# intel/hexl

Measured on NVIDIA H100. Metric: ntt_per_sec_fwd_inv_N65536_q55_batch8192, higher is better.
Workload: dtype u64

## Files before the change

### hexl_b200/csrc/ntt.cu

```cuda
#include "ntt_kernels.cuh"

namespace hexl_b200 {
namespace {

template <int MODE, int LOGC>
cudaError_t launch_row(bool fwd, const NttDeviceTables& t, u64* result, const u64* operand,
                       u64 batch, int out_mf, int fold, cudaStream_t stream) {
  using Cfg = RowCfg<LOGC, MODE>;
  const unsigned rows_per_poly = (unsigned)(t.n >> LOGC);
  const u64 total_rows = batch * rows_per_poly;
  const unsigned grid = (unsigned)((total_rows + Cfg::ROWS - 1) / Cfg::ROWS);
  const Mod m = make_mod(t);
  if (fwd) {
    if (cudaError_t e = ensure_dynamic_smem<ntt_row_fwd<MODE, LOGC>>(Cfg::SMEM)) return e;
    ntt_row_fwd<MODE, LOGC><<<grid, Cfg::THREADS, Cfg::SMEM, stream>>>(result, operand, Tab<MODE>::fwd(t), m,
                                                                       total_rows, rows_per_poly, out_mf);
  } else {
    if (cudaError_t e = ensure_dynamic_smem<ntt_row_inv<MODE, LOGC>>(Cfg::SMEM)) return e;
    ntt_row_inv<MODE, LOGC><<<grid, Cfg::THREADS, Cfg::SMEM, stream>>>(
        result, operand, Tab<MODE>::inv(t), m, total_rows, rows_per_poly, out_mf, fold, Tab<MODE>::inv_n(t),
        Tab<MODE>::inv_n_w(t));
  }
  count_launch();
  return cudaGetLastError();
}

template <int MODE>
cudaError_t launch_row_dyn(int log_c, bool fwd, const NttDeviceTables& t, u64* result,
                           const u64* operand, u64 batch, int out_mf, int fold,
                           cudaStream_t stream) {
  switch (log_c) {
#define ROW_CASE(L) \
  case L: return launch_row<MODE, L>(fwd, t, result, operand, batch, out_mf, fold, stream);
    ROW_CASE(4) ROW_CASE(5) ROW_CASE(6) ROW_CASE(7) ROW_CASE(8) ROW_CASE(9) ROW_CASE(10)
    ROW_CASE(11) ROW_CASE(12) ROW_CASE(13)
#undef ROW_CASE
  }
  return cudaErrorInvalidValue;
}

template <int MODE, int LOGR>
cudaError_t launch_col(bool fwd, const NttDeviceTables& t, u64* result, const u64* operand,
                       u64 batch, int log_s, int out_mf, int fold, cudaStream_t stream) {
  const u64 total_cols = (batch << t.log_n) >> LOGR;
  const u64 cols_per_block = 1ull << (log_s - LOGR);
  const unsigned threads = (unsigned)(cols_per_block < 256 ? cols_per_block : 256);
  const unsigned grid = (unsigned)((total_cols + threads - 1) / threads);
  const Mod m = make_mod(t);
  if (fwd)
    ntt_col<MODE, LOGR, true><<<grid, threads, 0, stream>>>(result, operand, Tab<MODE>::fwd(t), m, t.log_n, log_s,
                                                            total_cols, out_mf, fold, Tab<MODE>::inv_n(t),
                                                            Tab<MODE>::inv_n_w(t));
  else
    ntt_col<MODE, LOGR, false><<<grid, threads, 0, stream>>>(result, operand, Tab<MODE>::inv(t), m, t.log_n, log_s,
                                                             total_cols, out_mf, fold, Tab<MODE>::inv_n(t),
                                                             Tab<MODE>::inv_n_w(t));
  count_launch();
  return cudaGetLastError();
}

template <int MODE>
cudaError_t launch_col_dyn(int log_r, bool fwd, const NttDeviceTables& t, u64* result,
                           const u64* operand, u64 batch, int log_s, int out_mf, int fold,
                           cudaStream_t stream) {
  switch (log_r) {
    case 3: return launch_col<MODE, 3>(fwd, t, result, operand, batch, log_s, out_mf, fold, stream);
    case 4: return launch_col<MODE, 4>(fwd, t, result, operand, batch, log_s, out_mf, fold, stream);
  }
  if constexpr (MODE != kSmall)
    if (log_r == 5) return launch_col<MODE, 5>(fwd, t, result, operand, batch, log_s, out_mf, fold, stream);
  return cudaErrorInvalidValue;
}

cudaError_t simple_transform(bool fwd, const NttDeviceTables& t, u64* result, const u64* operand,
                             int out_mf, u64 batch, cudaStream_t stream) {
  const u64 total = batch << (t.log_n - 1);
  const unsigned threads = 128, grid = (unsigned)((total + threads - 1) / threads);
  const u64* src = operand;
  const Mod m = make_mod(t);
  for (int k = 0; k < t.log_n; ++k) {
    const int s = fwd ? k : t.log_n - 1 - k;
    const int last = k == t.log_n - 1;
    if (fwd)
      ntt_stage_simple<true><<<grid, threads, 0, stream>>>(result, src, t.fwd, m, t.log_n, s, total,
                                                           out_mf, last, t.inv_n, t.inv_n_w);
    else
      ntt_stage_simple<false><<<grid, threads, 0, stream>>>(result, src, t.inv, m, t.log_n, s, total,
                                                            out_mf, last, t.inv_n, t.inv_n_w);
    count_launch();
    src = result;
  }
  return cudaGetLastError();
}

template <int MODE, int LOGR>
cudaError_t launch_fused(bool fwd, const NttDeviceTables& t, u64* result, const u64* operand, u64 batch,
                         int out_mf, cudaStream_t stream) {
  using Cfg = FusedCfg<LOGR>;
  const Mod m = make_mod(t);
  cudaLaunchConfig_t cfg = {};
  cfg.gridDim = dim3((unsigned)(batch * Cfg::K));
  cfg.blockDim = dim3(Cfg::THREADS);
  cfg.dynamicSmemBytes = Cfg::SMEM;
  cfg.stream = stream;
  cudaLaunchAttribute attr;
  attr.id = cudaLaunchAttributeClusterDimension;
  attr.val.clusterDim.x = Cfg::K;
  attr.val.clusterDim.y = 1;
  attr.val.clusterDim.z = 1;
  cfg.attrs = &attr;
  cfg.numAttrs = 1;
  cudaError_t e;
  if (fwd)
    e = cudaLaunchKernelEx(&cfg, ntt_fused_fwd<MODE, LOGR>, result, operand, Tab<MODE>::fwd(t), m, out_mf);
  else
    e = cudaLaunchKernelEx(&cfg, ntt_fused_inv<MODE, LOGR>, result, operand, Tab<MODE>::inv(t), m, out_mf,
                           Tab<MODE>::inv_n(t), Tab<MODE>::inv_n_w(t));
  count_launch();
  return e != cudaSuccess ? e : cudaGetLastError();
}

template <int MODE, int LOGR>
cudaError_t launch_pipe(const NttDeviceTables& t, u64* result, const u64* operand, u64 batch, int out_mf,
                        cudaStream_t stream) {
  return launch_pipelined<ntt_pipe_fwd<MODE, LOGR>, PipeCfg<LOGR>>(batch, stream, result, operand, Tab<MODE>::fwd(t),
                                                                  make_mod(t), out_mf);
}

template <int MODE, int LOGR>
cudaError_t launch_dsmem(bool fwd, const NttDeviceTables& t, u64* result, const u64* operand, u64 batch, int out_mf,
                         cudaStream_t stream) {
  using Cfg = DsmemCfg<LOGR, MODE>;
  const Mod m = make_mod(t);
  cudaLaunchConfig_t cfg = {};
  cfg.gridDim = dim3((unsigned)(batch * Cfg::K));
  cfg.blockDim = dim3(Cfg::THREADS);
  cfg.dynamicSmemBytes = Cfg::SMEM;
  cfg.stream = stream;
  cudaLaunchAttribute attr;
  attr.id = cudaLaunchAttributeClusterDimension;
  attr.val.clusterDim.x = Cfg::K;
  attr.val.clusterDim.y = 1;
  attr.val.clusterDim.z = 1;
  cfg.attrs = &attr;
  cfg.numAttrs = 1;
  cudaError_t e;
  if (fwd) {
    if ((e = ensure_dynamic_smem<ntt_dsmem_fwd<MODE, LOGR>>(Cfg::SMEM)) != cudaSuccess) return e;
    e = cudaLaunchKernelEx(&cfg, ntt_dsmem_fwd<MODE, LOGR>, result, operand, Tab<MODE>::fwd(t), m, out_mf);
  } else {
    if ((e = ensure_dynamic_smem<ntt_dsmem_inv<MODE, LOGR>>(Cfg::SMEM)) != cudaSuccess) return e;
    e = cudaLaunchKernelEx(&cfg, ntt_dsmem_inv<MODE, LOGR>, result, operand, Tab<MODE>::inv(t), m, out_mf,
                           Tab<MODE>::inv_n(t), Tab<MODE>::inv_n_w(t));
  }
  count_launch();
  return e != cudaSuccess ? e : cudaGetLastError();
}

enum : int { kSplit, kPipe, kFused, kDsmem };
struct SinglePass {
  int kernel, log_r;
};
template <int MODE>
SinglePass plan_single_pass(int log_n, u64 batch, bool forward) {
  const int lr = log_n - 12;
  if (lr < 2 || lr > 5) return {kSplit, 0};
  if (MODE == kSmall) return {kDsmem, lr};
  if (forward && lr >= 3 && batch >= 64 && batch < (1ull << 31)) return {kPipe, lr};
  if (lr <= 3) return {kDsmem, lr};
  if (lr == 4) return {kFused, lr};
  return {kSplit, 0};
}

template <int MODE>
cudaError_t launch_single_pass(SinglePass p, bool fwd, const NttDeviceTables& t, u64* result, const u64* operand,
                               u64 batch, int out_mf, cudaStream_t stream) {
  if constexpr (MODE == kSmall) {
    switch (p.log_r) {
      case 2: return launch_dsmem<MODE, 2>(fwd, t, result, operand, batch, out_mf, stream);
      case 3: return launch_dsmem<MODE, 3>(fwd, t, result, operand, batch, out_mf, stream);
      case 4: return launch_dsmem<MODE, 4>(fwd, t, result, operand, batch, out_mf, stream);
      case 5: return launch_dsmem<MODE, 5>(fwd, t, result, operand, batch, out_mf, stream);
    }
  } else if (p.kernel == kPipe && fwd) {
    switch (p.log_r) {
      case 3: return launch_pipe<MODE, 3>(t, result, operand, batch, out_mf, stream);
      case 4: return launch_pipe<MODE, 4>(t, result, operand, batch, out_mf, stream);
      case 5: return launch_pipe<MODE, 5>(t, result, operand, batch, out_mf, stream);
    }
  } else if (p.kernel == kFused && p.log_r == 4) {
    return launch_fused<MODE, 4>(fwd, t, result, operand, batch, out_mf, stream);
  } else if (p.kernel == kDsmem) {
    switch (p.log_r) {
      case 2: return launch_dsmem<MODE, 2>(fwd, t, result, operand, batch, out_mf, stream);
      case 3: return launch_dsmem<MODE, 3>(fwd, t, result, operand, batch, out_mf, stream);
    }
  }
  return cudaErrorInvalidValue;
}

template <int MODE>
cudaError_t forward_impl(const NttDeviceTables& t, u64* result, const u64* operand, int out_mf,
                         u64 batch, cudaStream_t stream) {
  const SinglePass sp = plan_single_pass<MODE>(t.log_n, batch, true);
  if (sp.kernel != kSplit) return launch_single_pass<MODE>(sp, true, t, result, operand, batch, out_mf, stream);
  const int log_c = pick_row_log(t.log_n);
  int radices[8];
  const int ncol = plan_col_passes(t.log_n - log_c, radices);
  const u64* src = operand;
  int log_s = t.log_n;
  for (int p = 0; p < ncol; ++p) {
    cudaError_t e = launch_col_dyn<MODE>(radices[p], true, t, result, src, batch, log_s, out_mf, 0, stream);
    if (e != cudaSuccess) return e;
    log_s -= radices[p];
    src = result;
  }
  return launch_row_dyn<MODE>(log_c, true, t, result, src, batch, out_mf, 0, stream);
}

template <int MODE>
cudaError_t inverse_impl(const NttDeviceTables& t, u64* result, const u64* operand, int out_mf,
                         u64 batch, cudaStream_t stream) {
  const SinglePass sp = plan_single_pass<MODE>(t.log_n, batch, false);
  if (sp.kernel != kSplit) return launch_single_pass<MODE>(sp, false, t, result, operand, batch, out_mf, stream);
  const int log_c = pick_row_log(t.log_n);
  int radices[8];
  const int ncol = plan_col_passes(t.log_n - log_c, radices);
  cudaError_t e = launch_row_dyn<MODE>(log_c, false, t, result, operand, batch, out_mf, ncol == 0, stream);
  if (e != cudaSuccess) return e;
  int log_s = log_c;
  for (int p = ncol - 1; p >= 0; --p) {
    log_s += radices[p];
    e = launch_col_dyn<MODE>(radices[p], false, t, result, result, batch, log_s, out_mf, p == 0, stream);
    if (e != cudaSuccess) return e;
  }
  return cudaSuccess;
}

}

cudaError_t launch_ntt_forward(const NttDeviceTables& t, u64* result, const u64* operand,
                               int , int out_mf, u64 batch, cudaStream_t stream) {
  if (batch == 0) return cudaSuccess;
  if (t.log_n < 4) return simple_transform(true, t, result, operand, out_mf, batch, stream);
  switch (pick_mode(t.q)) {
    case kFast: return forward_impl<kFast>(t, result, operand, out_mf, batch, stream);
    case kSmall: return forward_impl<kSmall>(t, result, operand, out_mf, batch, stream);
    case kWide: return forward_impl<kWide>(t, result, operand, out_mf, batch, stream);
  }
  return forward_impl<kGeneric>(t, result, operand, out_mf, batch, stream);
}

cudaError_t launch_ntt_inverse(const NttDeviceTables& t, u64* result, const u64* operand,
                               int , int out_mf, u64 batch, cudaStream_t stream) {
  if (batch == 0) return cudaSuccess;
  if (t.log_n < 4) return simple_transform(false, t, result, operand, out_mf, batch, stream);
  switch (pick_mode(t.q)) {
    case kFast: return inverse_impl<kFast>(t, result, operand, out_mf, batch, stream);
    case kSmall: return inverse_impl<kSmall>(t, result, operand, out_mf, batch, stream);
    case kWide: return inverse_impl<kWide>(t, result, operand, out_mf, batch, stream);
  }
  return inverse_impl<kGeneric>(t, result, operand, out_mf, batch, stream);
}

}
```

### hexl_b200/csrc/ntt_kernels.cuh

```cuda
#pragma once
#include <algorithm>
#include <atomic>
#include <cstdio>
#include <cstdlib>

#include "internal.h"

namespace hexl_b200 {
namespace {

template <int I>
struct Idx {
  __host__ __device__ constexpr operator int() const { return I; }
};
template <int BEGIN, int END, typename F>
__device__ __forceinline__ void static_for(F&& f) {
  if constexpr (BEGIN < END) {
    f(Idx<BEGIN>{});
    static_for<BEGIN + 1, END>(f);
  }
}

enum : int { kGeneric = 0, kFast = 1, kSmall = 2, kWide = 3 };

// ... 453 lines not shown
template <int POLICY>
__device__ __forceinline__ void st_coef(u64* p, u64 v) {
  if (POLICY == kViaL2)
    __stcg(p, v);
  else
    __stcs(p, v);
}

template <int POLICY, typename E>
__device__ __forceinline__ E ld_row(const void* base, unsigned u0, unsigned off) {
  const unsigned idx = u0 + off;
  if constexpr (POLICY == kSmemRow)
    return static_cast<const E*>(base)[idx];
  else if constexpr (POLICY == kSmemRowPad)
    return static_cast<const E*>(base)[idx + (idx >> 4)];
  else
    return (E)ld_coef<POLICY>(static_cast<const u64*>(base) + u0 + off);
}
template <int POLICY, typename E>
__device__ __forceinline__ void st_row(void* base, unsigned u0, unsigned off, E v) {
  const unsigned idx = u0 + off;
  if constexpr (POLICY == kSmemRow)
    static_cast<E*>(base)[idx] = v;
  else if constexpr (POLICY == kSmemRowPad)
    static_cast<E*>(base)[idx + (idx >> 4)] = v;
  else
    st_coef<POLICY>(static_cast<u64*>(base) + u0 + off, v);
}

struct MirrorList {
  u64* const* p;
  unsigned count;
  u64 off;
};

template <int MODE, int LOGC, int LD, int ST>
__device__ __forceinline__ void row_fwd_body(void* out, const void* in, typename Ar<MODE>::E* srow, unsigned u,
                                             u64 base, const typename Ar<MODE>::Tw* __restrict__ tw, const Mod& m,
                                             int out_mf, bool active, typename Ar<MODE>::Tw* cta_stab = nullptr,
                                             bool reduce_in = false) {
  using E = typename Ar<MODE>::E;
  using Tw = typename Ar<MODE>::Tw;
  E v[16];
  constexpr int LB0 = LOGC - 4;
  Tw* stab = cta_stab ? cta_stab : reinterpret_cast<Tw*>(srow + row_elems<E>(LOGC));
  const unsigned u_in = reg_index<LB0>(u, 0);
  static_for<0, 16>([&](auto I) { constexpr int e = I; v[e] = ld_row<LD, E>(in, u_in, e << LB0); });
  if constexpr (LD < kSmemRow && sizeof(E) == 8) {
    if (reduce_in) {
      static_for<0, 16>([&](auto I) { constexpr int e = I; v[e] = reduce_any(v[e], m); });
    }
  }
  if constexpr (RowCfg<LOGC>::TW_TABLES) {
    if (cta_stab)
      load_row_twiddles<LOGC>(stab, threadIdx.x, blockDim.x, base, tw);
    else
      load_row_twiddles<LOGC>(stab, u, (1u << LOGC) / 16, base, tw);
    __syncthreads();
  }
  reg_stages<MODE, LOGC, LB0, LOGC - 1, LB0, true>(v, u, base, tw, stab, m, false, Tw{}, Tw{});
  fwd_passes<MODE, LOGC, 1>(v, srow, u, base, tw, stab, m);
  static_for<0, 16>([&](auto I) { constexpr int e = I; v[e] = fwd_out<MODE>(v[e], m, out_mf); });
  constexpr int LB_OUT = LB0 < 4 ? LB0 : 4;
  if constexpr (LOGC > 4) smem_exchange<0, LB_OUT>(v, srow, u);
  if (active) {
    const unsigned u_out = reg_index<LB_OUT>(u, 0);
    static_for<0, 16>([&](auto I) { constexpr int e = I; st_row<ST, E>(out, u_out, e << LB_OUT, v[e]); });
  }
}

template <int MODE, int LOGC, int LD, int ST>
__device__ __forceinline__ void row_inv_body(void* out, const void* in, typename Ar<MODE>::E* srow, unsigned u,
                                             u64 base, const typename Ar<MODE>::Tw* __restrict__ tw, const Mod& m,
                                             int out_mf, bool fold, typename Ar<MODE>::Tw inv_n,
                                             typename Ar<MODE>::Tw inv_n_w, bool active,
                                             typename Ar<MODE>::Tw* cta_stab = nullptr, const MirrorList* mir = nullptr,
                                             const ProdIn* prod = nullptr) {
  using Cfg = RowCfg<LOGC>;
  using E = typename Ar<MODE>::E;
  using Tw = typename Ar<MODE>::Tw;
  E v[16];
  constexpr int LB0 = LOGC - 4;
  constexpr int LB_IN = LB0 < 4 ? LB0 : 4;
  Tw* stab = cta_stab ? cta_stab : reinterpret_cast<Tw*>(srow + row_elems<E>(LOGC));
  const unsigned u_in = reg_index<LB_IN>(u, 0);
  static_for<0, 16>([&](auto I) { constexpr int e = I; v[e] = ld_row<LD, E>(in, u_in, e << LB_IN); });
  if constexpr (LD < kSmemRow && sizeof(E) == 8) {
    if (prod) {
      static_for<0, 16>([&](auto I) {
        constexpr int e = I;
        v[e] = prod_lazy<MODE>(v[e], ld_coef<LD>(prod->b + reg_index<LB_IN>(u, e)), m, prod->mu, prod->shift);
      });
    }
  }
  if constexpr (Cfg::TW_TABLES) {
    if (cta_stab)
      load_row_twiddles<LOGC>(stab, threadIdx.x, blockDim.x, base, tw);
    else
      load_row_twiddles<LOGC>(stab, u, (1u << LOGC) / 16, base, tw);
    __syncthreads();
  }
  if constexpr (LOGC > 4) smem_exchange<LB_IN, 0>(v, srow, u);
  inv_passes<MODE, LOGC, Cfg::PASSES - 1>(v, srow, u, base, tw, stab, m, fold, inv_n, inv_n_w);
  if (active) {
    static_for<0, 16>([&](auto I) {
      constexpr int e = I;
      st_row<ST, E>(out, reg_index<LB0>(u, 0), e << LB0, fold ? inv_out<MODE>(v[e], m, out_mf) : v[e]);
    });
    if (mir && fold) {
      for (unsigned p = 0; p < mir->count; ++p) {
        static_for<0, 16>([&](auto I) {
          constexpr int e = I;
          mir->p[p][mir->off + reg_index<LB0>(u, e)] = (u64)inv_out<MODE>(v[e], m, out_mf);
        });
      }
    }
  }
}

template <int MODE, int LOGC>
__global__ void __launch_bounds__(RowCfg<LOGC, MODE>::THREADS, RowCfg<LOGC, MODE>::MIN_BLOCKS)
    ntt_row_fwd(u64* result, const u64* operand, const typename Ar<MODE>::Tw* __restrict__ tw, const Mod m,
                u64 total_rows, unsigned rows_per_poly, int out_mf) {
  using Cfg = RowCfg<LOGC, MODE>;
  extern __shared__ __align__(16) unsigned char smem[];
  const unsigned row_local = threadIdx.x / Cfg::T, u = threadIdx.x % Cfg::T;
  u64 row = (u64)blockIdx.x * Cfg::ROWS + row_local;
  const bool active = row < total_rows;
  if (!active) row = total_rows - 1;
  const u64 base = (u64)rows_per_poly + (row % rows_per_poly);
  typename Cfg::Tw* cta_stab = nullptr;
  if (MODE == kSmall && Cfg::ROWS > 1 && Cfg::TW_TABLES && rows_per_poly == 1)
    cta_stab = reinterpret_cast<typename Cfg::Tw*>(smem + (size_t)row_elems<typename Cfg::E>(LOGC) * sizeof(typename Cfg::E));
  row_fwd_body<MODE, LOGC, kStream, kStream>(
      result + row * Cfg::C, operand + row * Cfg::C,
      reinterpret_cast<typename Cfg::E*>(smem + (size_t)row_local * Cfg::ROW_BYTES), u, base, tw, m, out_mf, active,
      cta_stab);
}

template <int MODE, int LOGC>
__global__ void __launch_bounds__(RowCfg<LOGC, MODE>::THREADS, RowCfg<LOGC, MODE>::MIN_BLOCKS)
    ntt_row_inv(u64* result, const u64* operand, const typename Ar<MODE>::Tw* __restrict__ tw, const Mod m,
                u64 total_rows, unsigned rows_per_poly, int out_mf, int fold, typename Ar<MODE>::Tw inv_n,
                typename Ar<MODE>::Tw inv_n_w) {
  using Cfg = RowCfg<LOGC, MODE>;
  extern __shared__ __align__(16) unsigned char smem[];
  const unsigned row_local = threadIdx.x / Cfg::T, u = threadIdx.x % Cfg::T;
  u64 row = (u64)blockIdx.x * Cfg::ROWS + row_local;
  const bool active = row < total_rows;
  if (!active) row = total_rows - 1;
  const u64 base = (u64)rows_per_poly + (row % rows_per_poly);
  typename Cfg::Tw* cta_stab = nullptr;
  if (MODE == kSmall && Cfg::ROWS > 1 && Cfg::TW_TABLES && rows_per_poly == 1)
    cta_stab = reinterpret_cast<typename Cfg::Tw*>(smem + (size_t)row_elems<typename Cfg::E>(LOGC) * sizeof(typename Cfg::E));
  row_inv_body<MODE, LOGC, kStream, kStream>(
      result + row * Cfg::C, operand + row * Cfg::C,
      reinterpret_cast<typename Cfg::E*>(smem + (size_t)row_local * Cfg::ROW_BYTES), u, base, tw, m, out_mf,
      fold != 0, inv_n, inv_n_w, active, cta_stab);
}

template <int MODE, int LOGR, bool FWD>
__device__ __forceinline__ void col_stages(typename Ar<MODE>::E (&v)[1 << LOGR], const typename Ar<MODE>::Tw* stw,
                                           const Mod& m, bool root_fold, typename Ar<MODE>::Tw inv_n,
                                           typename Ar<MODE>::Tw inv_n_w) {
  using E = typename Ar<MODE>::E;
  using Tw = typename Ar<MODE>::Tw;
  constexpr int R = 1 << LOGR;
  static_for<0, LOGR>([&](auto STEP) {
    constexpr int step = STEP;
    constexpr int s = FWD ? step : LOGR - 1 - step;
    constexpr int eb = LOGR - 1 - s;
    const E cq = stage_cq<MODE>(step, m);
    auto groups = [&] {
      static_for<0, (1 << s)>([&](auto GI) {
        constexpr int gi = GI;
        const Tw w = stw[(1 << s) + gi];
        static_for<0, (1 << eb)>([&](auto L) {
          constexpr int e = (gi << (eb + 1)) | L;
          if constexpr (FWD)
            fwd_bfly<MODE>(v[e], v[e | (1 << eb)], w, m);
          else
            inv_bfly<MODE>(v[e], v[e | (1 << eb)], w, m, cq);
        });
      });
    };
    if constexpr (!FWD && s == 0) {
      if (root_fold) {
        static_for<0, (1 << eb)>([&](auto L) {
          constexpr int l = L;
          inv_bfly_last<MODE>(v[l], v[l | (1 << eb)], inv_n, inv_n_w, m, cq);
        });
      } else {
        groups();
      }
    } else {
      groups();
    }
  });
  if constexpr (!FWD && MODE == kFast) {
    if (!root_fold) inv_pass_fixup<LOGR, R>(v, m);
  }
}

template <int MODE, int LOGR, bool FWD, int LD, int ST>
__device__ __forceinline__ void col_body(u64* result, const u64* operand, u64 off, int log_stride,
                                         const typename Ar<MODE>::Tw* stw, const Mod& m, int out_mf, bool root_fold,
                                         typename Ar<MODE>::Tw inv_n, typename Ar<MODE>::Tw inv_n_w,
                                         const MirrorList* mir = nullptr, bool reduce_in = false) {
  using E = typename Ar<MODE>::E;
  constexpr int R = 1 << LOGR;
  E v[R];
  static_for<0, R>([&](auto I) {
    constexpr int e = I;
    v[e] = (E)ld_coef<LD>(operand + off + ((u64)e << log_stride));
  });
  if constexpr (FWD && sizeof(E) == 8) {
    if (reduce_in) {
      static_for<0, R>([&](auto I) { constexpr int e = I; v[e] = reduce_any(v[e], m); });
    }
  }
  col_stages<MODE, LOGR, FWD>(v, stw, m, root_fold, inv_n, inv_n_w);
  const bool final_out = !FWD && root_fold;
  static_for<0, R>([&](auto I) {
    constexpr int e = I;
    st_coef<ST>(result + off + ((u64)e << log_stride), final_out ? inv_out<MODE>(v[e], m, out_mf) : v[e]);
  });
  if (mir && final_out) {
    for (unsigned p = 0; p < mir->count; ++p) {
      static_for<0, R>([&](auto I) {
        constexpr int e = I;
        mir->p[p][mir->off + off + ((u64)e << log_stride)] = (u64)inv_out<MODE>(v[e], m, out_mf);
      });
    }
  }
}

template <int MODE, int LOGR, bool FWD>
__global__ void __launch_bounds__(256)
    ntt_col(u64* result, const u64* operand, const typename Ar<MODE>::Tw* __restrict__ tw, const Mod m, int log_n,
            int log_s, u64 total_cols, int out_mf, int fold, typename Ar<MODE>::Tw inv_n,
            typename Ar<MODE>::Tw inv_n_w) {
  constexpr int R = 1 << LOGR;
  __shared__ typename Ar<MODE>::Tw stw[R];
  const int log_cols = log_s - LOGR;
  const u64 g0 = (u64)blockIdx.x * blockDim.x;
  const u64 blk = g0 >> log_cols;
  const u64 blocks_per_poly = 1ull << (log_n - log_s);
  const u64 base = blocks_per_poly + (blk & (blocks_per_poly - 1));
  for (int l = threadIdx.x; l < R; l += blockDim.x) {
    if (l == 0) continue;
    const int s = 31 - __clz(l);
    stw[l] = ld_tw(tw + (base << s) + (l - (1 << s)));
  }
  __syncthreads();
  const u64 g = g0 + threadIdx.x;
  if (g >= total_cols) return;
  const u64 c = g & ((1ull << log_cols) - 1);
  col_body<MODE, LOGR, FWD, kStream, kStream>(result, operand, (blk << log_s) + c, log_cols, stw, m, out_mf,
                                              !FWD && fold && log_s == log_n, inv_n, inv_n_w);
}

__device__ __forceinline__ void cluster_barrier() {
  asm volatile("barrier.cluster.arrive.release.aligned;\n\tbarrier.cluster.wait.acquire.aligned;" ::: "memory");
}

template <int LOGR>
struct FusedCfg {
  static constexpr int LOGC = 12, C = 1 << LOGC, R = 1 << LOGR;
  static constexpr int K = R < 8 ? R : 8;
  static constexpr int THREADS = 256;
  static constexpr int MIN_BLOCKS = LOGR <= 4 ? kRowMinBlocks : 2;
  static constexpr size_t SMEM = RowCfg<LOGC>::ROW_BYTES;
};

template <int MODE, int LOGR>
__global__ void __launch_bounds__(FusedCfg<LOGR>::THREADS, FusedCfg<LOGR>::MIN_BLOCKS)
    ntt_fused_fwd(u64* result, const u64* operand, const typename Ar<MODE>::Tw* __restrict__ tw, const Mod m,
                  int out_mf) {
  using Cfg = FusedCfg<LOGR>;
  using E = typename Ar<MODE>::E;
  using Tw = typename Ar<MODE>::Tw;
  extern __shared__ __align__(16) unsigned char smem_raw[];
  E* smem = reinterpret_cast<E*>(smem_raw);
  __shared__ Tw stw[Cfg::R];
  const unsigned rank = blockIdx.x % Cfg::K;
  const u64 poly_off = (u64)(blockIdx.x / Cfg::K) << (Cfg::LOGC + LOGR);
  for (int l = threadIdx.x; l < Cfg::R; l += Cfg::THREADS)
    if (l) stw[l] = ld_tw(tw + l);
  __syncthreads();
  constexpr int COLS = Cfg::C / Cfg::K;
#pragma unroll 1
  for (int c = threadIdx.x; c < COLS; c += Cfg::THREADS)
    col_body<MODE, LOGR, true, kStream, kViaL2>(result, operand, poly_off + rank * COLS + c, Cfg::LOGC, stw, m,
                                                out_mf, false, Tw{}, Tw{});
  cluster_barrier();
#pragma unroll 1
  for (unsigned r = rank; r < Cfg::R; r += Cfg::K) {
    u64* row = result + poly_off + (u64)r * Cfg::C;
    row_fwd_body<MODE, Cfg::LOGC, kViaL2, kStream>(row, row, smem, threadIdx.x, (u64)Cfg::R + r, tw, m, out_mf, true);
    if (r + Cfg::K < Cfg::R) __syncthreads();
  }
}

template <int MODE, int LOGR>
__global__ void __launch_bounds__(FusedCfg<LOGR>::THREADS, FusedCfg<LOGR>::MIN_BLOCKS)
    ntt_fused_inv(u64* result, const u64* operand, const typename Ar<MODE>::Tw* __restrict__ tw, const Mod m,
                  int out_mf, typename Ar<MODE>::Tw inv_n, typename Ar<MODE>::Tw inv_n_w) {
  using Cfg = FusedCfg<LOGR>;
  using E = typename Ar<MODE>::E;
  using Tw = typename Ar<MODE>::Tw;
  extern __shared__ __align__(16) unsigned char smem_raw[];
  E* smem = reinterpret_cast<E*>(smem_raw);
  __shared__ Tw stw[Cfg::R];
  const unsigned rank = blockIdx.x % Cfg::K;
  const u64 poly_off = (u64)(blockIdx.x / Cfg::K) << (Cfg::LOGC + LOGR);
  for (int l = threadIdx.x; l < Cfg::R; l += Cfg::THREADS)
    if (l) stw[l] = ld_tw(tw + l);
#pragma unroll 1
  for (unsigned r = rank; r < Cfg::R; r += Cfg::K) {
    const u64 off = poly_off + (u64)r * Cfg::C;
    row_inv_body<MODE, Cfg::LOGC, kStream, kViaL2>(result + off, operand + off, smem, threadIdx.x, (u64)Cfg::R + r,
                                                   tw, m, out_mf, false, inv_n, inv_n_w, true);
    __syncthreads();
  }
  cluster_barrier();
  constexpr int COLS = Cfg::C / Cfg::K;
#pragma unroll 1
  for (int c = threadIdx.x; c < COLS; c += Cfg::THREADS)
    col_body<MODE, LOGR, false, kViaL2, kStream>(result, result, poly_off + rank * COLS + c, Cfg::LOGC, stw, m,
                                                 out_mf, true, inv_n, inv_n_w);
}

__device__ __forceinline__ unsigned ld_acquire_gpu(const unsigned* p) {
  unsigned v;
  asm volatile("ld.acquire.gpu.global.u32 %0, [%1];" : "=r"(v) : "l"(p) : "memory");
  return v;
}
__device__ __forceinline__ void red_release_gpu(unsigned* p, unsigned v) {
  asm volatile("red.release.gpu.global.add.u32 [%0], %1;" ::"l"(p), "r"(v) : "memory");
}

template <int LOGR>
struct PipeCfg {
  static constexpr int LOGC = 12, C = 1 << LOGC, R = 1 << LOGR;
  static constexpr int THREADS = 256;
  static constexpr int CT = C / THREADS;
  static constexpr int SLOTS = CT + R;
  static constexpr int MIN_BLOCKS = FusedCfg<LOGR>::MIN_BLOCKS;
  static constexpr size_t SMEM = RowCfg<LOGC>::ROW_BYTES;
};

template <int MODE, int LOGR>
__global__ void __launch_bounds__(PipeCfg<LOGR>::THREADS, PipeCfg<LOGR>::MIN_BLOCKS)
    ntt_pipe_fwd(u64* result, const u64* operand, const typename Ar<MODE>::Tw* __restrict__ tw, const Mod m,
                 int out_mf, unsigned batch, unsigned lookahead, unsigned* counter, unsigned* done) {
  using Cfg = PipeCfg<LOGR>;
  using E = typename Ar<MODE>::E;
  using Tw = typename Ar<MODE>::Tw;
  extern __shared__ __align__(16) unsigned char smem_raw[];
  E* smem = reinterpret_cast<E*>(smem_raw);
  __shared__ Tw stw[Cfg::R];
  __shared__ unsigned s_item;
  for (int l = threadIdx.x; l < Cfg::R; l += Cfg::THREADS)
    if (l) stw[l] = ld_tw(tw + l);
  const unsigned total = (batch + lookahead) * Cfg::SLOTS;
  while (true) {
    __syncthreads();
    if (threadIdx.x == 0) s_item = atomicAdd(counter, 1u);
    __syncthreads();
    const unsigned item = s_item;
    if (item >= total) break;
    const unsigned blk = item / Cfg::SLOTS, j = item % Cfg::SLOTS;
    if (j < (unsigned)Cfg::CT) {
      if (blk >= batch) continue;
      const u64 poly_off = (u64)blk << (Cfg::LOGC + LOGR);
      col_body<MODE, LOGR, true, kStream, kViaL2>(result, operand, poly_off + j * Cfg::THREADS + threadIdx.x, Cfg::LOGC,
                                                  stw, m, out_mf, false, Tw{}, Tw{});
      __syncthreads();
      if (threadIdx.x == 0) red_release_gpu(done + blk, 1u);
    } else {
      if (blk < lookahead) continue;
      const unsigned p = blk - lookahead, r = j - Cfg::CT;
      if (threadIdx.x == 0)
        while (ld_acquire_gpu(done + p) < (unsigned)Cfg::CT) __nanosleep(100);
      __syncthreads();
      u64* row = result + ((u64)p << (Cfg::LOGC + LOGR)) + (u64)r * Cfg::C;
      row_fwd_body<MODE, Cfg::LOGC, kViaL2, kStream>(row, row, smem, threadIdx.x, (u64)Cfg::R + r, tw, m, out_mf, true);
    }
  }
}

__device__ __forceinline__ unsigned dsmem_address(const void* local_smem, unsigned cta_rank) {
  const unsigned a = (unsigned)__cvta_generic_to_shared(local_smem);
  unsigned r;
  asm("mapa.shared::cluster.u32 %0, %1, %2;" : "=r"(r) : "r"(a), "r"(cta_rank));
  return r;
}
__device__ __forceinline__ void dsmem_store(unsigned addr, unsigned v) {
  asm volatile("st.shared::cluster.u32 [%0], %1;" ::"r"(addr), "r"(v) : "memory");
}
__device__ __forceinline__ void dsmem_store(unsigned addr, u64 v) {
  asm volatile("st.shared::cluster.u64 [%0], %1;" ::"r"(addr), "l"(v) : "memory");
}
template <typename E>
__device__ __forceinline__ E dsmem_load(unsigned addr) {
  E v;
  if constexpr (sizeof(E) == 8)
    asm volatile("ld.shared::cluster.u64 %0, [%1];" : "=l"(v) : "r"(addr) : "memory");
  else
    asm volatile("ld.shared::cluster.u32 %0, [%1];" : "=r"(v) : "r"(addr) : "memory");
  return v;
}

template <int LOGR, int MODE = kSmall>
struct DsmemCfg {
  using E = typename Ar<MODE>::E;
  using Tw = typename Ar<MODE>::Tw;
  static constexpr int LOGC = 12, C = 1 << LOGC, R = 1 << LOGR;
  static constexpr int K = R < 8 ? R : 8;
  static constexpr int RPC = R / K;
  static constexpr int THREADS = 256;
  static constexpr int COLS = C / K;
  static constexpr bool PAD = sizeof(E) == 8;
  static constexpr int ROW_POLICY = PAD ? kSmemRowPad : kSmemRow;
  static constexpr unsigned ROW = row_elems<E>(LOGC);
  static constexpr size_t SMEM = (size_t)(RPC + (PAD ? 0 : 1)) * ROW * sizeof(E) + kRowTwEntries * sizeof(Tw);
  static constexpr int MIN_BLOCKS = PAD ? kRowMinBlocks : (SMEM <= 56 * 1024 ? 4 : (SMEM <= 75 * 1024 ? 3 : 2));
  static __device__ __forceinline__ unsigned slot(unsigned j) { return PAD ? j + (j >> 4) : j; }
};

template <int MODE, int LOGR>
__global__ void __launch_bounds__(DsmemCfg<LOGR, MODE>::THREADS, DsmemCfg<LOGR, MODE>::MIN_BLOCKS)
    ntt_dsmem_fwd(u64* result, const u64* operand, const typename Ar<MODE>::Tw* __restrict__ tw, const Mod m,
                  int out_mf) {
  using Cfg = DsmemCfg<LOGR, MODE>;
  using E = typename Ar<MODE>::E;
  using Tw = typename Ar<MODE>::Tw;
  extern __shared__ __align__(16) unsigned char smem_raw[];
  E* rows = reinterpret_cast<E*>(smem_raw);
  E* xbuf = rows + Cfg::RPC * Cfg::ROW;
  Tw* const ctab = Cfg::PAD ? reinterpret_cast<Tw*>(xbuf) : nullptr;
  __shared__ Tw stw[Cfg::R];
  const unsigned rank = blockIdx.x % Cfg::K;
  const u64 poly_off = (u64)(blockIdx.x / Cfg::K) << (Cfg::LOGC + LOGR);
  asm volatile("barrier.cluster.arrive.relaxed.aligned;" ::: "memory");
  for (int l = threadIdx.x; l < Cfg::R; l += Cfg::THREADS)
    if (l) stw[l] = ld_tw(tw + l);
  __syncthreads();
  asm volatile("barrier.cluster.wait.aligned;" ::: "memory");
  unsigned owner_base[Cfg::K];
  static_for<0, Cfg::K>([&](auto I) { constexpr int o = I; owner_base[o] = dsmem_address(rows, o); });
#pragma unroll 1
  for (int c = threadIdx.x; c < Cfg::COLS; c += Cfg::THREADS) {
    const unsigned col = rank * Cfg::COLS + c;
    E v[Cfg::R];
    static_for<0, Cfg::R>([&](auto I) {
      constexpr int e = I;
      v[e] = (E)ld_coef<kStream>(operand + poly_off + ((u64)e << Cfg::LOGC) + col);
    });
    col_stages<MODE, LOGR, true>(v, stw, m, false, Tw{}, Tw{});
    static_for<0, Cfg::R>([&](auto I) {
      constexpr int e = I;
      dsmem_store(owner_base[e % Cfg::K] + ((e / Cfg::K) * Cfg::ROW + Cfg::slot(col)) * (unsigned)sizeof(E), v[e]);
    });
  }
  cluster_barrier();
#pragma unroll 1
  for (int lr = 0; lr < Cfg::RPC; ++lr) {
    const unsigned r = rank + lr * Cfg::K;
    E* row = rows + lr * Cfg::ROW;
    row_fwd_body<MODE, Cfg::LOGC, Cfg::ROW_POLICY, kStream>(result + poly_off + (u64)r * Cfg::C, row,
                                                            Cfg::PAD ? row : xbuf, threadIdx.x, (u64)Cfg::R + r, tw, m,
                                                            out_mf, true, ctab);
    if (lr + 1 < Cfg::RPC) __syncthreads();
  }
}

template <int MODE, int LOGR>
__global__ void __launch_bounds__(DsmemCfg<LOGR, MODE>::THREADS, DsmemCfg<LOGR, MODE>::MIN_BLOCKS)
    ntt_dsmem_inv(u64* result, const u64* operand, const typename Ar<MODE>::Tw* __restrict__ tw, const Mod m,
                  int out_mf, typename Ar<MODE>::Tw inv_n, typename Ar<MODE>::Tw inv_n_w) {
  using Cfg = DsmemCfg<LOGR, MODE>;
  using E = typename Ar<MODE>::E;
  using Tw = typename Ar<MODE>::Tw;
  extern __shared__ __align__(16) unsigned char smem_raw[];
  E* rows = reinterpret_cast<E*>(smem_raw);
  E* xbuf = rows + Cfg::RPC * Cfg::ROW;
  Tw* const ctab = Cfg::PAD ? reinterpret_cast<Tw*>(xbuf) : nullptr;
  __shared__ Tw stw[Cfg::R];
  const unsigned rank = blockIdx.x % Cfg::K;
  const u64 poly_off = (u64)(blockIdx.x / Cfg::K) << (Cfg::LOGC + LOGR);
  for (int l = threadIdx.x; l < Cfg::R; l += Cfg::THREADS)
    if (l) stw[l] = ld_tw(tw + l);
#pragma unroll 1
  for (int lr = 0; lr < Cfg::RPC; ++lr) {
    const unsigned r = rank + lr * Cfg::K;
    E* row = rows + lr * Cfg::ROW;
    row_inv_body<MODE, Cfg::LOGC, kStream, Cfg::ROW_POLICY>(row, operand + poly_off + (u64)r * Cfg::C,
                                                            Cfg::PAD ? row : xbuf, threadIdx.x, (u64)Cfg::R + r, tw, m,
                                                            out_mf, false, inv_n, inv_n_w, true, ctab);
    __syncthreads();
  }
  cluster_barrier();
  unsigned owner_base[Cfg::K];
  static_for<0, Cfg::K>([&](auto I) { constexpr int o = I; owner_base[o] = dsmem_address(rows, o); });
#pragma unroll 1
  for (int c = threadIdx.x; c < Cfg::COLS; c += Cfg::THREADS) {
    const unsigned col = rank * Cfg::COLS + c;
    E v[Cfg::R];
    static_for<0, Cfg::R>([&](auto I) {
      constexpr int e = I;
      v[e] = dsmem_load<E>(owner_base[e % Cfg::K] + ((e / Cfg::K) * Cfg::ROW + Cfg::slot(col)) * (unsigned)sizeof(E));
    });
    col_stages<MODE, LOGR, false>(v, stw, m, true, inv_n, inv_n_w);
    static_for<0, Cfg::R>([&](auto I) {
      constexpr int e = I;
      st_coef<kStream>(result + poly_off + ((u64)e << Cfg::LOGC) + col, inv_out<MODE>(v[e], m, out_mf));
    });
  }
  cluster_barrier();
}

template <bool FWD>
__global__ void ntt_stage_simple(u64* result, const u64* src, const Twiddle* __restrict__ tw,
                                 const Mod m, int log_n, int s ,
                                 u64 total_bflies, int out_mf, int last, Twiddle inv_n,
                                 Twiddle inv_n_w) {
  const u64 g = (u64)blockIdx.x * blockDim.x + threadIdx.x;
  if (g >= total_bflies) return;
  const int log_t = log_n - 1 - s;
  const u64 half = 1ull << (log_n - 1);
  const u64 poly = g >> (log_n - 1), k = g & (half - 1);
  const u64 i = k >> log_t, jj = k & ((1ull << log_t) - 1);
  const u64 j = (poly << log_n) + (i << (log_t + 1)) + jj;
  u64 X = src[j], Y = src[j + (1ull << log_t)];
  if (FWD) {
    fwd_bfly<kGeneric>(X, Y, ld_tw(tw + (1ull << s) + i), m);
    if (last) {
      X = fwd_out<kGeneric>(X, m, out_mf);
      Y = fwd_out<kGeneric>(Y, m, out_mf);
    }
  } else if (last) {
    inv_bfly_last<kGeneric>(X, Y, inv_n, inv_n_w, m, m.two_q);
    X = inv_out<kGeneric>(X, m, out_mf);
    Y = inv_out<kGeneric>(Y, m, out_mf);
  } else {
    inv_bfly<kGeneric>(X, Y, ld_tw(tw + (1ull << s) + i), m, m.two_q);
  }
  result[j] = X;
  result[j + (1ull << log_t)] = Y;
}


template <auto Kernel>
cudaError_t ensure_dynamic_smem(size_t bytes) {
  if (bytes <= 48 * 1024) return cudaSuccess;
  static std::atomic<unsigned long long> done{0};
  int dev = 0;
  cudaGetDevice(&dev);
  const unsigned long long bit = 1ull << (dev & 63);
  if (done.load(std::memory_order_acquire) & bit) return cudaSuccess;
  const cudaError_t e = cudaFuncSetAttribute(Kernel, cudaFuncAttributeMaxDynamicSharedMemorySize, (int)bytes);
  if (e == cudaSuccess) done.fetch_or(bit, std::memory_order_release);
  return e;
}

template <auto Kernel, typename Cfg, typename... Args>
cudaError_t launch_pipelined(u64 units, cudaStream_t stream, Args... args) {
  static const unsigned lookahead = [] {
    const char* v = std::getenv("HEXL_B200_PIPE_LOOKAHEAD");
    return (unsigned)std::max(1, v ? std::atoi(v) : 16);
  }();
  cudaError_t e = ensure_dynamic_smem<Kernel>(Cfg::SMEM);
  if (e != cudaSuccess) return e;
  int dev = 0, sms = 0;
  cudaGetDevice(&dev);
  cudaDeviceGetAttribute(&sms, cudaDevAttrMultiProcessorCount, dev);
  const u64 items = (units + lookahead) * Cfg::SLOTS;
  const unsigned grid = (unsigned)std::min<u64>((u64)sms * Cfg::MIN_BLOCKS, items);
  unsigned* state = nullptr;
  const size_t bytes = (size_t)(units + 1) * sizeof(unsigned);
  if ((e = scratch_alloc_async(reinterpret_cast<void**>(&state), bytes, stream)) != cudaSuccess) return e;
  if ((e = cudaMemsetAsync(state, 0, bytes, stream)) == cudaSuccess) {
    Kernel<<<grid, Cfg::THREADS, Cfg::SMEM, stream>>>(args..., (unsigned)units, lookahead, state, state + 1);
    count_launch();
    e = cudaGetLastError();
  }
  scratch_free_async(state, stream);
  return e;
}

inline int pick_mode(u64 q) {
  if (q < kSmallModulusLimit) return kSmall;
  if (q < kFastModulusLimit && q >= (1ull << 32)) return kFast;
  return (q >= kFastModulusLimit && q < kWideModulusLimit) ? kWide : kGeneric;
}

template <int MODE>
struct Tab {
  static const Twiddle* fwd(const NttDeviceTables& t) { return t.fwd; }
  static const Twiddle* inv(const NttDeviceTables& t) { return t.inv; }
  static Twiddle inv_n(const NttDeviceTables& t) { return t.inv_n; }
  static Twiddle inv_n_w(const NttDeviceTables& t) { return t.inv_n_w; }
};
template <>
struct Tab<kSmall> {
  static const Twiddle32* fwd(const NttDeviceTables& t) { return t.fwd32; }
  static const Twiddle32* inv(const NttDeviceTables& t) { return t.inv32; }
  static Twiddle32 inv_n(const NttDeviceTables& t) { return t.inv_n32; }
  static Twiddle32 inv_n_w(const NttDeviceTables& t) { return t.inv_n_w32; }
};

__host__ __device__ inline Mod make_mod(u64 q, u64 mu) {
  Mod m;
  m.q = q;
  m.two_q = q << 1;
  m.four_q = q << 2;
  m.mu = mu;
  const u64 negq = 0 - q;
  m.n0 = (unsigned)negq;
  m.n1 = (unsigned)(negq >> 32);
  m.zero = 0;
  return m;
}
inline Mod make_mod(const NttDeviceTables& t) { return make_mod(t.q, t.mu); }

inline int plan_col_passes(int top_stages, int out[8]) {
  if (top_stages <= 0) return 0;
  const int passes = (top_stages + 4) / 5;
  int left = top_stages;
  for (int p = 0; p < passes; ++p) {
    out[p] = (left + (passes - p) - 1) / (passes - p);
    left -= out[p];
  }
  return passes;
}


}
}
```

Before: 1.463 million.

## Replace cluster-based fused inverse NTT with persistent pipelined work-queue kernel

The inverse fused NTT no longer runs as one cluster per polynomial with a cluster barrier between its row and column phases. It now uses a persistent-grid kernel that pulls work items from an atomic counter. Row items for one polynomial overlap with column items for an earlier polynomial, and completion is tracked with release/acquire counters, using twice the forward lookahead. This aims to hide the barrier stall and the tail imbalance between phases, at the cost of atomic traffic, spin-waiting, and a static_assert that requires SLOTS to be a power of two.

```diff
diff --git a/hexl_b200/csrc/ntt.cu b/hexl_b200/csrc/ntt.cu
--- a/hexl_b200/csrc/ntt.cu
+++ b/hexl_b200/csrc/ntt.cu
@@ -98,6 +98,10 @@
                          int out_mf, cudaStream_t stream) {
   using Cfg = FusedCfg<LOGR>;
   const Mod m = make_mod(t);
+  if (!fwd)
+    return launch_pipelined<ntt_fused_inv<MODE, LOGR>, PipeCfg<LOGR>, 2>(batch, stream, result, operand,
+                                                                        Tab<MODE>::inv(t), m, out_mf,
+                                                                        Tab<MODE>::inv_n(t), Tab<MODE>::inv_n_w(t));
   cudaLaunchConfig_t cfg = {};
   cfg.gridDim = dim3((unsigned)(batch * Cfg::K));
   cfg.blockDim = dim3(Cfg::THREADS);
@@ -110,12 +114,8 @@
   attr.val.clusterDim.z = 1;
   cfg.attrs = &attr;
   cfg.numAttrs = 1;
-  cudaError_t e;
-  if (fwd)
-    e = cudaLaunchKernelEx(&cfg, ntt_fused_fwd<MODE, LOGR>, result, operand, Tab<MODE>::fwd(t), m, out_mf);
-  else
-    e = cudaLaunchKernelEx(&cfg, ntt_fused_inv<MODE, LOGR>, result, operand, Tab<MODE>::inv(t), m, out_mf,
-                           Tab<MODE>::inv_n(t), Tab<MODE>::inv_n_w(t));
+  const cudaError_t e =
+      cudaLaunchKernelEx(&cfg, ntt_fused_fwd<MODE, LOGR>, result, operand, Tab<MODE>::fwd(t), m, out_mf);
   count_launch();
   return e != cudaSuccess ? e : cudaGetLastError();
 }
diff --git a/hexl_b200/csrc/ntt_kernels.cuh b/hexl_b200/csrc/ntt_kernels.cuh
--- a/hexl_b200/csrc/ntt_kernels.cuh
+++ b/hexl_b200/csrc/ntt_kernels.cuh
@@ -779,35 +779,6 @@
   }
 }
 
-template <int MODE, int LOGR>
-__global__ void __launch_bounds__(FusedCfg<LOGR>::THREADS, FusedCfg<LOGR>::MIN_BLOCKS)
-    ntt_fused_inv(u64* result, const u64* operand, const typename Ar<MODE>::Tw* __restrict__ tw, const Mod m,
-                  int out_mf, typename Ar<MODE>::Tw inv_n, typename Ar<MODE>::Tw inv_n_w) {
-  using Cfg = FusedCfg<LOGR>;
-  using E = typename Ar<MODE>::E;
-  using Tw = typename Ar<MODE>::Tw;
-  extern __shared__ __align__(16) unsigned char smem_raw[];
-  E* smem = reinterpret_cast<E*>(smem_raw);
-  __shared__ Tw stw[Cfg::R];
-  const unsigned rank = blockIdx.x % Cfg::K;
-  const u64 poly_off = (u64)(blockIdx.x / Cfg::K) << (Cfg::LOGC + LOGR);
-  for (int l = threadIdx.x; l < Cfg::R; l += Cfg::THREADS)
-    if (l) stw[l] = ld_tw(tw + l);
-#pragma unroll 1
-  for (unsigned r = rank; r < Cfg::R; r += Cfg::K) {
-    const u64 off = poly_off + (u64)r * Cfg::C;
-    row_inv_body<MODE, Cfg::LOGC, kStream, kViaL2>(result + off, operand + off, smem, threadIdx.x, (u64)Cfg::R + r,
-                                                   tw, m, out_mf, false, inv_n, inv_n_w, true);
-    __syncthreads();
-  }
-  cluster_barrier();
-  constexpr int COLS = Cfg::C / Cfg::K;
-#pragma unroll 1
-  for (int c = threadIdx.x; c < COLS; c += Cfg::THREADS)
-    col_body<MODE, LOGR, false, kViaL2, kStream>(result, result, poly_off + rank * COLS + c, Cfg::LOGC, stw, m,
-                                                 out_mf, true, inv_n, inv_n_w);
-}
-
 __device__ __forceinline__ unsigned ld_acquire_gpu(const unsigned* p) {
   unsigned v;
   asm volatile("ld.acquire.gpu.global.u32 %0, [%1];" : "=r"(v) : "l"(p) : "memory");
@@ -867,6 +838,48 @@
   }
 }
 
+template <int MODE, int LOGR>
+__global__ void __launch_bounds__(PipeCfg<LOGR>::THREADS, PipeCfg<LOGR>::MIN_BLOCKS)
+    ntt_fused_inv(u64* result, const u64* operand, const typename Ar<MODE>::Tw* __restrict__ tw, const Mod m,
+                  int out_mf, typename Ar<MODE>::Tw inv_n, typename Ar<MODE>::Tw inv_n_w, unsigned batch,
+                  unsigned lookahead, unsigned* counter, unsigned* done) {
+  using Cfg = PipeCfg<LOGR>;
+  using E = typename Ar<MODE>::E;
+  using Tw = typename Ar<MODE>::Tw;
+  static_assert((Cfg::SLOTS & (Cfg::SLOTS - 1)) == 0, "the item split is a shift and a mask");
+  extern __shared__ __align__(16) unsigned char smem_raw[];
+  E* smem = reinterpret_cast<E*>(smem_raw);
+  __shared__ Tw stw[Cfg::R];
+  __shared__ unsigned s_item;
+  for (int l = threadIdx.x; l < Cfg::R; l += Cfg::THREADS)
+    if (l) stw[l] = ld_tw(tw + l);
+  const unsigned total = (batch + lookahead) * Cfg::SLOTS;
+  while (true) {
+    __syncthreads();
+    if (threadIdx.x == 0) s_item = atomicAdd(counter, 1u);
+    __syncthreads();
+    const unsigned item = s_item;
+    if (item >= total) break;
+    const unsigned blk = item / Cfg::SLOTS, j = item % Cfg::SLOTS;
+    if (j < (unsigned)Cfg::R) {
+      if (blk >= batch) continue;
+      const u64 off = ((u64)blk << (Cfg::LOGC + LOGR)) + ((u64)j << Cfg::LOGC);
+      row_inv_body<MODE, Cfg::LOGC, kStream, kViaL2>(result + off, operand + off, smem, threadIdx.x, (u64)Cfg::R + j,
+                                                     tw, m, out_mf, false, inv_n, inv_n_w, true);
+      __syncthreads();
+      if (threadIdx.x == 0) red_release_gpu(done + blk, 1u);
+    } else {
+      if (blk < lookahead) continue;
+      const unsigned p = blk - lookahead, c = j - Cfg::R;
+      if (threadIdx.x == 0)
+        while (ld_acquire_gpu(done + p) < (unsigned)Cfg::R) __nanosleep(100);
+      __syncthreads();
+      col_body<MODE, LOGR, false, kViaL2, kStream>(result, result, ((u64)p << (Cfg::LOGC + LOGR)) + c * Cfg::THREADS +
+                                                   threadIdx.x, Cfg::LOGC, stw, m, out_mf, true, inv_n, inv_n_w);
+    }
+  }
+}
+
 __device__ __forceinline__ unsigned dsmem_address(const void* local_smem, unsigned cta_rank) {
   const unsigned a = (unsigned)__cvta_generic_to_shared(local_smem);
   unsigned r;
@@ -1042,9 +1055,9 @@
   return e;
 }
 
-template <auto Kernel, typename Cfg, typename... Args>
+template <auto Kernel, typename Cfg, unsigned SCALE = 1, typename... Args>
 cudaError_t launch_pipelined(u64 units, cudaStream_t stream, Args... args) {
-  static const unsigned lookahead = [] {
+  static const unsigned lookahead = SCALE * [] {
     const char* v = std::getenv("HEXL_B200_PIPE_LOOKAHEAD");
     return (unsigned)std::max(1, v ? std::atoi(v) : 16);
   }();
```

Result: faster. 1.486 million (median of 6 runs) (+1.5%).
